# ishine/minimax-speech

Measured on NVIDIA B200. Metric: audio-sec synthesized/sec (24 kHz), higher is better.
Workload: dtype bf16

## Files before the change

minimax-speech_b200/csrc/kernels.h:

```cpp
#pragma once
#include <atomic>
#include <cstdint>
#include <cuda.h>
#include <cuda_bf16.h>
#include <cuda_runtime.h>

namespace ls {

extern std::atomic<long long> g_launch_count;
extern long long* g_debug_buffer;
extern long long g_debug_bytes;
inline void count_launch() { g_launch_count.fetch_add(1, std::memory_order_relaxed); }

bool pdl_enabled();
bool conv_halo_enabled();
int conv_halo_mode();
bool conv_fuse_res_enabled();
bool conv_dual_enabled();
bool conv_resident_enabled();
bool conv_tma_out_enabled();
template <typename... KArgs, typename... Args>
inline cudaError_t launch_pdl(void (*kernel)(KArgs...), dim3 grid, dim3 block, size_t smem, cudaStream_t stream,
                              int cluster, Args&&... args) {
  cudaLaunchConfig_t cfg = {};
// ... 85 lines not shown
cudaError_t launch_conv_gemm_fp16(const CUtensorMap& mapA0, const CUtensorMap& mapA1, const CUtensorMap& mapW,
                                  const ConvGemmParams& p, int num_sms, cudaStream_t stream);

#ifndef ATTN_KV
#define ATTN_KV 64
#endif
struct AttnParams {
  int B, T, H;
  const int* lengths;
  int chunk;
  float scale_log2e;
  __nv_bfloat16* out;
  const float* bias;
  long long bias_ld, bias_bh;
  long long* timeline;
  long long timeline_entries;
  int fp16;
};
cudaError_t launch_attention(const CUtensorMap& mapQKV, const AttnParams& p, cudaStream_t stream);
cudaError_t launch_attention_fp16(const CUtensorMap& mapQKV, const AttnParams& p, cudaStream_t stream);

#define TBLOCK_VEC_FLOATS 2560
#ifndef TBLOCK_PAIR
#define TBLOCK_PAIR 0
#endif
#if TBLOCK_PAIR
#undef TBLOCK_CLUSTER
#define TBLOCK_CLUSTER 2
#endif
#ifndef TBLOCK_CLUSTER
#define TBLOCK_CLUSTER 1
#endif
#define TBLOCK_WBOX_ROWS (128 / TBLOCK_CLUSTER)
#define TBLOCK_WIDE_BOX_ROWS (TBLOCK_PAIR ? 128 : TBLOCK_WBOX_ROWS)
struct TBlockParams {
  int R;
  int T;
  const int* lengths;
  const float* vec;
  int tail_mode;
  long long* timeline;
  int fp16;
  int no_skip;
};
struct TBlockMaps {
  CUtensorMap att;
  CUtensorMap wo, w1, w2, wqkv;
// ... 47 lines not shown
```

minimax-speech_b200/csrc/ptx.cuh:

```cuda
#pragma once
#include <cstdint>
#include <cuda.h>
#include <cuda_bf16.h>
#include <cuda_fp16.h>
#include <cuda_runtime.h>

#ifndef LS_HALF_FP16
#define LS_HALF_FP16 0
#endif

namespace ls {

__device__ __forceinline__ uint32_t smem_u32(const void* p) {
  return static_cast<uint32_t>(__cvta_generic_to_shared(p));
}

__device__ __forceinline__ void mbar_init(uint64_t* bar, uint32_t count) {
  asm volatile("mbarrier.init.shared::cta.b64 [%0], %1;" ::"r"(smem_u32(bar)), "r"(count) : "memory");
}
__device__ __forceinline__ void fence_barrier_init() {
  asm volatile("fence.mbarrier_init.release.cluster;" ::: "memory");
}
__device__ __forceinline__ void mbar_arrive_expect_tx(uint64_t* bar, uint32_t bytes) {
  asm volatile("mbarrier.arrive.expect_tx.shared::cta.b64 _, [%0], %1;" ::"r"(smem_u32(bar)), "r"(bytes)
// ... 21 lines not shown
#ifdef LS_WAIT_SLEEP_NS
    __nanosleep(LS_WAIT_SLEEP_NS);
#endif
    if ((++spins & 0x3FFu) == 0 && clock64() - t0 > 4000000000LL) __trap();
  }
}

__device__ __forceinline__ void pdl_launch_dependents() { asm volatile("griddepcontrol.launch_dependents;" ::: "memory"); }
__device__ __forceinline__ void pdl_wait() { asm volatile("griddepcontrol.wait;" ::: "memory"); }

template <int N>
__device__ __forceinline__ void reg_dealloc() { asm volatile("setmaxnreg.dec.sync.aligned.u32 %0;" ::"n"(N)); }
template <int N>
__device__ __forceinline__ void reg_alloc() { asm volatile("setmaxnreg.inc.sync.aligned.u32 %0;" ::"n"(N)); }

__device__ __forceinline__ void prefetch_tmap(const CUtensorMap* m) {
  asm volatile("prefetch.tensormap [%0];" ::"l"(reinterpret_cast<uint64_t>(m)) : "memory");
}
__device__ __forceinline__ void tma_prefetch_l2_2d(const CUtensorMap* m, int c0, int c1) {
  asm volatile("cp.async.bulk.prefetch.tensor.2d.L2.global.tile [%0, {%1, %2}];"
               ::"l"(reinterpret_cast<uint64_t>(m)), "r"(c0), "r"(c1)
               : "memory");
}
__device__ __forceinline__ void tma_load_2d(void* dst, const CUtensorMap* m, uint64_t* bar, int c0, int c1) {
  asm volatile(
      "cp.async.bulk.tensor.2d.shared::cluster.global.tile.mbarrier::complete_tx::bytes [%0], [%1, {%3, %4}], [%2];"
      ::"r"(smem_u32(dst)), "l"(reinterpret_cast<uint64_t>(m)), "r"(smem_u32(bar)), "r"(c0), "r"(c1)
      : "memory");
}
__device__ __forceinline__ void tma_load_3d(void* dst, const CUtensorMap* m, uint64_t* bar, int c0, int c1,
                                            int c2) {
  asm volatile(
      "cp.async.bulk.tensor.3d.shared::cluster.global.tile.mbarrier::complete_tx::bytes [%0], [%1, {%3, %4, %5}], [%2];"
      ::"r"(smem_u32(dst)), "l"(reinterpret_cast<uint64_t>(m)), "r"(smem_u32(bar)), "r"(c0), "r"(c1), "r"(c2)
      : "memory");
}
__device__ __forceinline__ void tma_load_2d_mc(void* dst, const CUtensorMap* m, uint64_t* bar, int c0, int c1,
                                               uint16_t cta_mask) {
  asm volatile(
      "cp.async.bulk.tensor.2d.shared::cluster.global.tile.mbarrier::complete_tx::bytes.multicast::cluster "
      "[%0], [%1, {%3, %4}], [%2], %5;"
      ::"r"(smem_u32(dst)), "l"(reinterpret_cast<uint64_t>(m)), "r"(smem_u32(bar)), "r"(c0), "r"(c1), "h"(cta_mask)
      : "memory");
}
__device__ __forceinline__ uint32_t cluster_ctarank() {
  uint32_t r;
// ... 82 lines not shown
               "h"(cta_mask)
               : "memory");
}
__device__ __forceinline__ void tmem_alloc_pair(uint32_t* dst_smem, uint32_t ncols) {
  asm volatile("tcgen05.alloc.cta_group::2.sync.aligned.shared::cta.b32 [%0], %1;" ::"r"(smem_u32(dst_smem)),
               "r"(ncols)
               : "memory");
}
__device__ __forceinline__ void tmem_relinquish_pair() {
  asm volatile("tcgen05.relinquish_alloc_permit.cta_group::2.sync.aligned;" ::: "memory");
}
__device__ __forceinline__ void tmem_dealloc_pair(uint32_t taddr, uint32_t ncols) {
  asm volatile("tcgen05.dealloc.cta_group::2.sync.aligned.b32 %0, %1;" ::"r"(taddr), "r"(ncols) : "memory");
}
__device__ __forceinline__ void umma_bf16_pair(uint32_t tmem_d, uint64_t adesc, uint64_t bdesc, uint32_t idesc,
                                               uint32_t accumulate) {
  asm volatile(
      "{\n\t.reg .pred p;\n\t"
      "setp.ne.b32 p, %4, 0;\n\t"
      "tcgen05.mma.cta_group::2.kind::f16 [%0], %1, %2, %3, p;\n\t}"
      ::"r"(tmem_d), "l"(adesc), "l"(bdesc), "r"(idesc), "r"(accumulate)
      : "memory");
}
__device__ __forceinline__ void umma_commit_pair(uint64_t* bar) {
  asm volatile("tcgen05.commit.cta_group::2.mbarrier::arrive::one.shared::cluster.multicast::cluster.b64 [%0], %1;" ::"r"(
                   smem_u32(bar)),
               "h"((uint16_t)3)
               : "memory");
}
__device__ __forceinline__ uint32_t cluster_addr(const void* p, uint32_t rank) {
  uint32_t r;
  asm volatile("mapa.shared::cluster.u32 %0, %1, %2;" : "=r"(r) : "r"(smem_u32(p)), "r"(rank));
  return r;
}
__device__ __forceinline__ void mbar_arrive_cluster(uint32_t bar_cluster_addr) {
  asm volatile("mbarrier.arrive.release.cluster.shared::cluster.b64 _, [%0];" ::"r"(bar_cluster_addr) : "memory");
}
__device__ __forceinline__ void mbar_arrive_expect_tx_cluster(uint32_t bar_cluster_addr, uint32_t bytes) {
  asm volatile("mbarrier.arrive.expect_tx.release.cluster.shared::cluster.b64 _, [%0], %1;" ::"r"(bar_cluster_addr),
               "r"(bytes)
               : "memory");
}
__device__ __forceinline__ void tma_load_2d_pair(void* dst, const CUtensorMap* m, uint32_t bar_cluster_addr, int c0, int c1) {
  asm volatile(
      "cp.async.bulk.tensor.2d.cta_group::2.shared::cluster.global.tile.mbarrier::complete_tx::bytes [%0], [%1, {%3, %4}], [%2];"
      ::"r"(smem_u32(dst)), "l"(reinterpret_cast<uint64_t>(m)), "r"(bar_cluster_addr), "r"(c0), "r"(c1)
      : "memory");
}
__device__ __forceinline__ void tma_load_3d_pair(void* dst, const CUtensorMap* m, uint32_t bar_cluster_addr, int c0, int c1,
                                                 int c2) {
  asm volatile(
      "cp.async.bulk.tensor.3d.cta_group::2.shared::cluster.global.tile.mbarrier::complete_tx::bytes [%0], [%1, {%3, %4, %5}], [%2];"
      ::"r"(smem_u32(dst)), "l"(reinterpret_cast<uint64_t>(m)), "r"(bar_cluster_addr), "r"(c0), "r"(c1), "r"(c2)
      : "memory");
}
__device__ __forceinline__ bool mbar_try_wait_cluster(uint64_t* bar, uint32_t parity) {
  uint32_t ok;
  asm volatile(
      "{\n\t.reg .pred p;\n\t"
      "mbarrier.try_wait.parity.acquire.cluster.shared::cta.b64 p, [%1], %2;\n\t"
      "selp.u32 %0, 1, 0, p;\n\t}"
      : "=r"(ok)
      : "r"(smem_u32(bar)), "r"(parity)
      : "memory");
  return ok != 0;
}
__device__ __forceinline__ void mbar_wait_cluster(uint64_t* bar, uint32_t parity) {
  const long long t0 = clock64();
  uint32_t spins = 0;
  while (!mbar_try_wait_cluster(bar, parity)) {
    if ((++spins & 0x3FFu) == 0 && clock64() - t0 > 4000000000LL) __trap();
  }
}
__device__ __forceinline__ void tmem_ld_wait() { asm volatile("tcgen05.wait::ld.sync.aligned;" ::: "memory"); }

__device__ __forceinline__ void tmem_ld16(uint32_t taddr, uint32_t (&r)[16]) {
  asm volatile(
      "tcgen05.ld.sync.aligned.32x32b.x16.b32 {%0,%1,%2,%3,%4,%5,%6,%7,%8,%9,%10,%11,%12,%13,%14,%15}, [%16];"
      : "=r"(r[0]), "=r"(r[1]), "=r"(r[2]), "=r"(r[3]), "=r"(r[4]), "=r"(r[5]), "=r"(r[6]), "=r"(r[7]),
        "=r"(r[8]), "=r"(r[9]), "=r"(r[10]), "=r"(r[11]), "=r"(r[12]), "=r"(r[13]), "=r"(r[14]), "=r"(r[15])
      : "r"(taddr)
      : "memory");
}
__device__ __forceinline__ void tmem_ld32(uint32_t taddr, uint32_t (&r)[32]) {
  asm volatile(
      "tcgen05.ld.sync.aligned.32x32b.x32.b32 "
      "{%0,%1,%2,%3,%4,%5,%6,%7,%8,%9,%10,%11,%12,%13,%14,%15,"
      "%16,%17,%18,%19,%20,%21,%22,%23,%24,%25,%26,%27,%28,%29,%30,%31}, [%32];"
      : "=r"(r[0]), "=r"(r[1]), "=r"(r[2]), "=r"(r[3]), "=r"(r[4]), "=r"(r[5]), "=r"(r[6]), "=r"(r[7]),
        "=r"(r[8]), "=r"(r[9]), "=r"(r[10]), "=r"(r[11]), "=r"(r[12]), "=r"(r[13]), "=r"(r[14]), "=r"(r[15]),
        "=r"(r[16]), "=r"(r[17]), "=r"(r[18]), "=r"(r[19]), "=r"(r[20]), "=r"(r[21]), "=r"(r[22]), "=r"(r[23]),
        "=r"(r[24]), "=r"(r[25]), "=r"(r[26]), "=r"(r[27]), "=r"(r[28]), "=r"(r[29]), "=r"(r[30]), "=r"(r[31])
      : "r"(taddr)
      : "memory");
}
// ... 154 lines not shown
```

minimax-speech_b200/csrc/tblock.cu:

```cuda
#include "kernels.h"
#include "profiler.h"
#include "ptx.cuh"

namespace ls {
namespace {

constexpr int kC = 256, kInner = 512, kFF = 1024, kQKV = 1536;
constexpr int kTileM = 128;
constexpr int kSlotBytes = 128 * 64 * 2;
constexpr bool kPair = TBLOCK_PAIR != 0;
constexpr int kRingSlotBytes = kSlotBytes;
#ifndef TBLOCK_SLOTS
#define TBLOCK_SLOTS 5
#endif
constexpr int kSlots = TBLOCK_SLOTS;
#ifndef TBLOCK_PRODUCER_WARPS
#define TBLOCK_PRODUCER_WARPS 3
#endif
constexpr int kProducerWarps = TBLOCK_PRODUCER_WARPS;
constexpr int kMmaWarp = kProducerWarps;
#ifndef TBLOCK_PRODUCER_LANES
#define TBLOCK_PRODUCER_LANES 1
#endif
constexpr int kProducerLanes = TBLOCK_PRODUCER_LANES;
constexpr int kIssuers = kProducerWarps * kProducerLanes;
static_assert(kIssuers <= kSlots, "interleaved producers must not outnumber the ring slots (parity waits)");
static_assert(!kPair || TBLOCK_CLUSTER == 2, "pair mode is a cluster of two");
constexpr int kCS = TBLOCK_CLUSTER;
constexpr int kPartRows = 128 / kCS;
constexpr int kPartBytes = kPartRows * 128;
constexpr uint16_t kCtaMask = (uint16_t)((1u << kCS) - 1);
#ifndef TBLOCK_RING_B
#define TBLOCK_RING_B 0
#endif
constexpr bool kRingB = TBLOCK_RING_B != 0 && !kPair && kCS == 1;
#ifndef TBLOCK_WIDE_FF
#define TBLOCK_WIDE_FF 0
#endif
#ifndef TBLOCK_FF2_TS
#define TBLOCK_FF2_TS 1
#endif
constexpr bool kFf2Ts = TBLOCK_FF2_TS != 0 && !kPair;
#ifndef TBLOCK_DETAIL_TL
#define TBLOCK_DETAIL_TL 0
#endif
constexpr bool kDetailTl = TBLOCK_DETAIL_TL != 0;
#ifndef TBLOCK_MERGE_ELECT
#define TBLOCK_MERGE_ELECT 0
#endif
constexpr bool kMergeElect = TBLOCK_MERGE_ELECT != 0;
#ifndef TBLOCK_L2_PREFETCH
#define TBLOCK_L2_PREFETCH 1
#endif
constexpr bool kL2Prefetch = TBLOCK_L2_PREFETCH != 0 && !kPair && kCS == 1;
#ifndef TBLOCK_ATT_DIRECT
#define TBLOCK_ATT_DIRECT 1
#endif
constexpr bool kAttDirect = TBLOCK_ATT_DIRECT != 0 && !kPair && kCS == 1 && !kRingB;
constexpr int kOutLoads = kAttDirect ? 16 : 24;
constexpr bool kWide = TBLOCK_WIDE_FF != 0 && kAttDirect && kFf2Ts && kSlots == 5 && !kMergeElect;
constexpr int kWideSlots = 9;
constexpr int kWideAhPerTile = 26;
static_assert(!kRingB || kFf2Ts, "the second ring lives in the AH region: it needs the TS form of FF2");
constexpr int kSlotsB = 4;
constexpr int kEpiWarps = 16;
constexpr int kEpiThreads = kEpiWarps * 32;
constexpr int kFirstEpiWarp = kProducerWarps + 1;
constexpr int kThreads = kFirstEpiWarp * 32 + kEpiThreads;

constexpr int kOffA3 = 0;
constexpr int kOffAH = 4 * kSlotBytes;
constexpr int kOffRing = kOffAH + 4 * kSlotBytes;
constexpr int kOffVec = kOffRing + kSlots * kRingSlotBytes;
constexpr int kOffRed = kOffVec + TBLOCK_VEC_FLOATS * 4;
constexpr int kOffBars = kOffRed + 4 * kTileM * 8;
constexpr int kBarBytes = 1024;
constexpr int kSmemBytes = kOffBars + kBarBytes + 1024;
static_assert(kSmemBytes <= 227 * 1024, "tblock shared memory budget");

constexpr int V_BO = 0, V_G3 = 256, V_BE3 = 512, V_B1 = 768, V_B2 = 1792, V_G1N = 2048, V_BE1N = 2304;
static_assert(V_BE1N + 256 == TBLOCK_VEC_FLOATS, "vector pack layout");

constexpr uint32_t kTmemD = 0, kTmemH = 256;
// ... 107 lines not shown
  const int n_groups = (n_tiles + kCS - 1) / kCS;
  const int group0 = blockIdx.x / kCS, group_step = gridDim.x / kCS;
  auto group_skipped = [&](int g) {
    for (int r = 0; r < kCS; ++r)
      if (!tile_all_padding(p, (g * kCS + r) * kTileM)) return false;
    return true;
  };
  long long* tl = p.timeline ? p.timeline + (size_t)blockIdx.x * 256 : nullptr;
#define TL(i)                         \
  do {                                \
    if (tl) tl[(i)] = clock64();      \
  } while (0)

  if (warp == 0 && lane == 0) {
    prefetch_tmap(&mapAtt);
    prefetch_tmap(&mapWo);
    prefetch_tmap(&mapW1);
    prefetch_tmap(&mapW2);
    prefetch_tmap(&mapWqkv);
    prefetch_tmap(&mapU);
    prefetch_tmap(&mapQkvOut);
    prefetch_tmap(&mapTail);
    for (int i = 0; i < kWideSlots; ++i) {
      mbar_init(&full[i], kPair ? 2 : 1);
      mbar_init(&empty[i], kPair ? 1 : kCS);
      mbar_init(&empty[kWideSlots + i], 1);
    }
    mbar_init(d_full, 1);
    mbar_init(a3_ready, kPair ? 2 * kEpiWarps : kEpiWarps);
    for (int i = 0; i < 2; ++i) {
      mbar_init(&h_full[i], 1);
      mbar_init(&ah_ready[i], kPair ? 2 * kEpiWarps : kEpiWarps);
      mbar_init(&ah_free[i], 1);
    }
    mbar_init(u_full, 1);
    for (int i = 0; i < kSlotsB; ++i) {
      mbar_init(&full_b[i], 1);
      mbar_init(&empty_b[i], 1);
    }
    mbar_init(stage_free, 1);
    for (int i = 0; i < 8; ++i) {
      mbar_init(&full_c[i], 1);
      mbar_init(&empty_c[i], 1);
    }
    fence_barrier_init();
  }
  if (kL2Prefetch && warp == 1 && lane == 0) {
    const int n_boxes = head ? 48 : (do_qkv ? 128 : 80);
    for (int j = blockIdx.x; j < n_boxes; j += gridDim.x) {
      int q = j;
      if (head || q >= 80) {
        if (!head) q -= 80;
        tma_prefetch_l2_2d(&mapWqkv, (q & 3) * 64, (q >> 2) * 128);
      } else if (q < 16) {
        tma_prefetch_l2_2d(&mapWo, (q >> 1) * 64, (q & 1) * 128);
      } else if (q < 48) {
        q -= 16;
        tma_prefetch_l2_2d(&mapW1, (q & 3) * 64, (q >> 2) * 128);
      } else {
        q -= 48;
        tma_prefetch_l2_2d(&mapW2, (q >> 1) * 64, (q & 1) * 128);
      }
    }
  }
  if (warp == kMmaWarp) {
    __syncwarp();
    if (kPair) {
      tmem_alloc_pair(tmem_slot, 512);
      tmem_relinquish_pair();
    } else {
      tmem_alloc(tmem_slot, 512);
      tmem_relinquish();
    }
  }
  if (warp >= kFirstEpiWarp) {
    for (int i = threadIdx.x - kFirstEpiWarp * 32; i < TBLOCK_VEC_FLOATS; i += kEpiThreads) sVec[i] = __ldg(p.vec + i);
  }
  pdl_launch_dependents();
  tc_fence_before();
  __syncthreads();
  if (kCS > 1) cluster_sync_all();
  tc_fence_after();
  const uint32_t tmem_base = *tmem_slot;
  pdl_wait();

  if (warp < kProducerWarps) {
    constexpr bool kWarpIssue = kProducerLanes == 1;
    if (kWarpIssue || lane < kProducerLanes) {
      const int issuer = warp * kProducerLanes + (kWarpIssue ? 0 : lane);
      const int per_tile = kPair ? (head ? 24 : (do_qkv ? 72 : 48)) : (head ? 48 : (do_qkv ? kOutLoads + 112 : kOutLoads + 64));
      long long seq0 = 0;
      uint32_t tile_n = 0;
      for (int g = group0; g < n_groups; g += group_step) {
        const int row0 = (g * kCS + rank) * kTileM;
        if (kWarpIssue ? __shfl_sync(0xffffffffu, (int)group_skipped(g), 0) != 0 : group_skipped(g)) continue;
        const bool two_rings = kRingB && !head;
        const bool b_warp = two_rings && warp == kProducerWarps - 1;
        const int n_a = two_rings ? kIssuers - kProducerLanes : kIssuers;
        for (int i = two_rings ? 0 : issuer; i < per_tile; i += two_rings ? 1 : kIssuers) {
          const CUtensorMap* m;
          int c0, c1;
          bool own_rows = false;
          int c2 = -1;
          int ring_b = -1, chunk_b = 0;
          int a_idx = i;
          if (kPair) {
            auto chunk_half = [&](const CUtensorMap* wm, int chunk, int half) {
              m = wm, c0 = 0, c1 = chunk * 128 + rank * kPartRows, c2 = half * 2;
            };
            if (head) {
              chunk_half(&mapWqkv, i >> 1, i & 1);
            } else if (i < 16) {
              const int kb = i >> 1;
              if ((i & 1) == 0) m = &mapAtt, c0 = kb * 64, c1 = row0, own_rows = true;
              else m = &mapWo, c0 = kb * 64, c1 = rank * 128, own_rows = true;
            } else if (i < 20) {
              chunk_half(&mapW1, (i - 16) >> 1, i & 1);
            } else if (i < 48) {
              const int j = i - 20;
              int c, r;
              if (j < 24) c = j >> 2, r = j & 3;
              else c = 6 + ((j - 24) >> 1), r = (j - 24) & 1;
              if (r < 2) m = &mapW2, c0 = c * 128 + r * 64, c1 = rank * 128, own_rows = true;
              else chunk_half(&mapW1, c + 2, r - 2);
            } else {
              chunk_half(&mapWqkv, (i - 48) >> 1, i & 1);
            }
          } else if (head) {
            m = &mapWqkv, c0 = (i & 3) * 64, c1 = (i >> 2) * 128;
          } else if (kAttDirect && i < kOutLoads) {
            m = &mapWo, c0 = (i >> 1) * 64, c1 = (i & 1) * 128;
          } else if (i < kOutLoads) {
            const int kb = i / 3, r = i - kb * 3;
            if (r == 0) m = &mapAtt, c0 = kb * 64, c1 = row0, own_rows = true;
            else m = &mapWo, c0 = kb * 64, c1 = (r - 1) * 128;
          } else if (i < kOutLoads + 8) {
            const int j = i - kOutLoads;
            m = &mapW1, c0 = (j & 3) * 64, c1 = (j >> 2) * 128;
          } else if (i < kOutLoads + 64) {
            const int j = i - (kOutLoads + 8);
            int c, r;
            if (j < 48) c = j >> 3, r = j & 7;
            else c = 6 + ((j - 48) >> 2), r = (j - 48) & 3;
            if (r < 4) {
              m = &mapW2, c0 = c * 128 + (r >> 1) * 64, c1 = (r & 1) * 128;
              if (kRingB) ring_b = r, chunk_b = c;
            } else {
              m = &mapW1, c0 = (r - 4) * 64, c1 = (c + 2) * 128;
            }
// ... 24 lines not shown
              if (hc < 4) mbar_wait(stage_free, tile_n & 1);
            } else {
              const uint32_t cnt = tile_n * (uint32_t)(per_tile - (head ? 0 : kWideAhPerTile)) + (uint32_t)rc;
              sl = 4 + (int)(cnt % 5u), use = cnt / 5u;
            }
            if (use > 0) mbar_wait(&empty[((use - 1) & 1) * kWideSlots + sl], ((use - 1) >> 1) & 1);
            if (tl && i < 48 && tile_n == 0 && (!kWarpIssue || lane == 0)) tl[64 + i] = clock64();
            full_bar = &full[sl];
            dst = sAH + sl * kSlotBytes;
          } else if (ring_b >= 0) {
            if (chunk_b == 0) mbar_wait(stage_free, tile_n & 1);
            else mbar_wait(&empty_b[ring_b], (tile_n * 7 + (uint32_t)chunk_b - 1) & 1);
            full_bar = &full_b[ring_b];
            dst = sAH + ring_b * kSlotBytes;
          } else {
            const long long seq = seq0 + a_idx;
            const int slot = (int)(seq % kSlots);
            const uint32_t use = (uint32_t)(seq / kSlots);
            mbar_wait(&empty[slot], (use & 1) ^ 1);
            if (tl && seq < 48 && (!kWarpIssue || lane == 0)) tl[64 + seq] = clock64();
            full_bar = &full[slot];
            dst = sRing + slot * kRingSlotBytes;
          }
          const int qk6 = kOutLoads + 64 + 24;
          const bool stamp_q6 = kDetailTl && tl && !kWide && do_qkv && !head && i >= qk6 && i < qk6 + 4 && seq0 == 0;
          if (stamp_q6 && (!kWarpIssue || lane == 0)) tl[216 + 2 * (i - qk6)] = clock64();
          if (kWarpIssue && !elect_one()) {
          } else if (kPair) {
            const uint32_t fb = cluster_addr(full_bar, 0);
            mbar_arrive_expect_tx_cluster(fb, kRingSlotBytes);
            if (c2 >= 0) tma_load_3d_pair(dst, m, fb, c0, c1, c2);
            else tma_load_2d_pair(dst, m, fb, c0, c1);
          } else {
            mbar_arrive_expect_tx(full_bar, kSlotBytes);
            if (kCS > 1 && !own_rows) tma_load_2d_mc(dst + rank * kPartBytes, m, full_bar, c0, c1 + rank * kPartRows, kCtaMask);
            else tma_load_2d(dst, m, full_bar, c0, c1);
          }
          if (kWarpIssue) __syncwarp();
          if (stamp_q6 && (!kWarpIssue || lane == 0)) tl[217 + 2 * (i - qk6)] = clock64();
        }
        seq0 += (kRingB && !head) ? per_tile - 32 : per_tile;
        tile_n += 1;
      }
    }
  } else if (warp == kMmaWarp) {
    if (!kPair || rank == 0) {
      const uint32_t tmem_u = __shfl_sync(0xffffffffu, tmem_base, 0);
#define TLM(i)                                 \
  do {                                         \
    if (tl && lane == 0) tl[(i)] = clock64();  \
  } while (0)
      const uint32_t idesc = make_idesc_bf16(kPair ? 2 * kTileM : kTileM, 128, false, false);
      const uint32_t idesc256 = make_idesc_bf16(2 * kTileM, 256, false, false);
      auto mma = [&](uint32_t d, uint64_t ad, uint64_t bd, uint32_t acc) {
        if (kPair) umma_bf16_pair(d, ad, bd, idesc, acc);
        else umma_bf16(d, ad, bd, idesc, acc);
      };
      auto commit = [&](uint64_t* bar) {
        if (elect_one()) {
          if (kPair) umma_commit_pair(bar);
          else umma_commit(bar);
        }
        __syncwarp();
      };
      auto wait_epi = [&](uint64_t* bar, uint32_t parity) {
        if (kPair) mbar_wait_cluster(bar, parity);
        else mbar_wait(bar, parity);
      };
      int slot = 0;
      uint32_t phase = 0;
      uint32_t a3_cnt = 0;
      uint32_t fills0 = 0, fills1 = 0;
      uint32_t drained0 = 0, drained1 = 0;
      int n_full = 0;
      uint32_t tile_n = 0;
      int r_slot = 0, h_slot = 0, f_pos = 0;
      uint32_t r_use = 0, h_use = 0;
      bool in_f = false;
      auto wide_peek = [&](int ahead, uint32_t& use) -> int {
        int rs = r_slot, hs = h_slot, fp = f_pos;
        uint32_t ru = r_use, hu = h_use;
        for (int a = 0;; ++a) {
          const bool ah = in_f && fp < 4;
          if (a == ahead) {
            use = ah ? hu : ru;
            return ah ? hs : 4 + rs;
          }
          if (ah) {
            if (++hs == 4) hs = 0, ++hu;
          } else {
            if (++rs == 5) rs = 0, ++ru;
// ... 4 lines not shown
      auto wide_advance = [&](int n) {
        for (int a = 0; a < n; ++a) {
          if (in_f && f_pos < 4) {
            if (++h_slot == 4) h_slot = 0, ++h_use;
          } else {
            if (++r_slot == 5) r_slot = 0, ++r_use;
          }
          if (in_f && ++f_pos == 9) f_pos = 0;
        }
      };
      auto slot_desc = [&](int ahead) -> uint64_t {
        if (kWide) {
          uint32_t use;
          const int sl = wide_peek(ahead, use);
          mbar_wait(&full[sl], use & 1);
          tc_fence_after();
          if (tl && lane == 0 && n_full < 16) tl[112 + n_full] = clock64();
          n_full += (ahead == 0);
          return make_smem_desc_sw128(smem_u32(sAH + sl * kSlotBytes));
        }
        int s = slot + ahead;
        uint32_t ph = phase;
        if (s >= kSlots) s -= kSlots, ph ^= 1;
        if (kPair) mbar_wait_cluster(&full[s], ph);
        else mbar_wait(&full[s], ph);
        tc_fence_after();
        if (tl && lane == 0 && n_full < 16) tl[112 + n_full] = clock64();
        n_full += (ahead == 0);
        return make_smem_desc_sw128(smem_u32(sRing + s * kRingSlotBytes));
      };
      auto release = [&](int n) {
        if (kWide) {
          if (elect_one()) {
            for (int j = 0; j < n; ++j) {
              uint32_t use;
              const int sl = wide_peek(j, use);
              umma_commit(&empty[(use & 1) * kWideSlots + sl]);
            }
          }
          __syncwarp();
          wide_advance(n);
          return;
        }
        if (elect_one()) {
          int sl = slot;
          for (int j = 0; j < n; ++j) {
            if (kPair) umma_commit_pair(&empty[sl]);
            else if (kCS > 1) umma_commit_mc(&empty[sl], kCtaMask);
// ... 2 lines not shown
          }
        }
        __syncwarp();
        for (int j = 0; j < n; ++j)
          if (++slot == kSlots) slot = 0, phase ^= 1;
      };
      auto release_elected = [&](int n) {
        int sl = slot;
        for (int j = 0; j < n; ++j) {
          if (kPair) umma_commit_pair(&empty[sl]);
          else if (kCS > 1) umma_commit_mc(&empty[sl], kCtaMask);
          else umma_commit(&empty[sl]);
          if (++sl == kSlots) sl = 0;
        }
      };
      auto advance = [&](int n) {
        __syncwarp();
        for (int j = 0; j < n; ++j)
          if (++slot == kSlots) slot = 0, phase ^= 1;
      };
      auto wait_drained = [&](int i) {
        const uint32_t f = i ? fills1 : fills0;
        if ((i ? drained1 : drained0) < f) {
          wait_epi(&ah_ready[i], (f - 1) & 1);
          tc_fence_after();
          if (i) drained1 = f;
          else drained0 = f;
        }
      };
      auto gemm_from_a3 = [&](int i, int tlb = -1) {
        if (kDetailTl && tl && tlb >= 0 && lane == 0) tl[tlb] = clock64();
        wait_drained(i);
        if (kDetailTl && tl && tlb >= 0 && lane == 0) tl[tlb + 1] = clock64();
        const uint32_t d = tmem_u + kTmemH + (uint32_t)i * 128;
        for (int kb = 0; kb < kC / 64; ++kb) {
          const uint64_t bdesc = slot_desc(0) + (kPair ? (uint64_t)((kb & 1) * (8192 >> 4)) : 0);
          if (kDetailTl && tl && tlb >= 0 && lane == 0) tl[tlb + 2 + kb] = clock64();
          const uint64_t adesc = make_smem_desc_sw128(smem_u32(sA3 + kb * kSlotBytes));
          if (kMergeElect && !kPair) {
            if (elect_one()) {
#pragma unroll
              for (int k = 0; k < 4; ++k) mma(d, adesc + 2 * k, bdesc + 2 * k, (kb | k) != 0 ? 1u : 0u);
              release_elected(1);
            }
            advance(1);
            continue;
          }
// ... 4 lines not shown
          if (kDetailTl && tl && tlb >= 0 && lane == 0) tl[tlb + 56 + 2 * kb] = clock64();
          if (!kPair || (kb & 1)) release(1);
          if (kDetailTl && tl && tlb >= 0 && lane == 0) tl[tlb + 57 + 2 * kb] = clock64();
        }
        commit(&h_full[i]);
        if (kDetailTl && tl && tlb >= 0 && lane == 0) tl[tlb + 6] = clock64();
        if (i) fills1 += 1;
        else fills0 += 1;
      };
      const uint32_t dD = tmem_u + kTmemD;
      TLM(0);
      for (int g = group0; g < n_groups; g += group_step, ++tile_n) {
        if (__shfl_sync(0xffffffffu, (int)group_skipped(g), 0)) {
          --tile_n;
          continue;
        }
        if (g != group0) tl = nullptr;
        if (!head) {
        for (int kb = 0; kb < kInner / 64; ++kb) {
          if (kAttDirect) {
            mbar_wait(&full_c[kb], tile_n & 1);
            tc_fence_after();
            const uint64_t adesc = make_smem_desc_sw128(smem_u32(att_place(kb)));
            const uint64_t b0 = slot_desc(0);
            const uint64_t b1 = slot_desc(1);
            if (kb == 0) TLM(1);
            if (elect_one()) {
#pragma unroll
              for (int k = 0; k < 4; ++k) {
                const uint32_t acc = (kb | k) != 0 ? 1u : 0u;
                mma(dD, adesc + 2 * k, b0 + 2 * k, acc);
                mma(dD + 128, adesc + 2 * k, b1 + 2 * k, acc);
              }
              if (!kWide) release_elected(2);
              umma_commit(&empty_c[kb]);
            }
            if (kWide) release(2);
            else advance(2);
            continue;
          }
          const uint64_t adesc = slot_desc(0);
          const uint64_t b0 = slot_desc(1);
          if (kPair) {
            if (kb == 0) TLM(1);
            if (elect_one()) {
#pragma unroll
              for (int k = 0; k < 4; ++k) umma_bf16_pair(dD, adesc + 2 * k, b0 + 2 * k, idesc256, (kb | k) != 0 ? 1u : 0u);
            }
            release(2);
            continue;
          }
          const uint64_t b1 = slot_desc(2);
          if (kb == 0) TLM(1);
          if (elect_one()) {
#pragma unroll
            for (int k = 0; k < 4; ++k) {
              const uint32_t acc = (kb | k) != 0 ? 1u : 0u;
              mma(dD, adesc + 2 * k, b0 + 2 * k, acc);
              mma(dD + 128, adesc + 2 * k, b1 + 2 * k, acc);
            }
            if (kMergeElect) release_elected(3);
          }
          if (kMergeElect) advance(3);
          else release(3);
        }
        commit(d_full);
        TLM(2);
        wait_epi(a3_ready, a3_cnt & 1);
        a3_cnt += 1;
        tc_fence_after();
        TLM(3);
        gemm_from_a3(0);
        gemm_from_a3(1);
        in_f = true, f_pos = 0;
        for (int c = 0; c < kFF / 128; ++c) {
          const int i = c & 1;
          if (kDetailTl && c == 4) TLM(128);
          wait_drained(i);
          TLM(4 + c);
          for (int kb2 = 0; kb2 < 2; ++kb2) {
            const uint32_t a_tm = tmem_u + kTmemH + (uint32_t)i * 128 + (uint32_t)kb2 * 64;
            const uint64_t adesc = make_smem_desc_sw128(smem_u32(sAH + i * 2 * kSlotBytes + kb2 * kSlotBytes));
            if (kPair) {
              const uint64_t b0 = slot_desc(0);
              if (elect_one()) {
#pragma unroll
                for (int k = 0; k < 4; ++k) umma_bf16_pair(dD, adesc + 2 * k, b0 + 2 * k, idesc256, 1u);
              }
              release(1);
              continue;
            }
            uint64_t b0, b1;
            if (kRingB) {
              const uint32_t par = (tile_n * 8 + (uint32_t)c) & 1;
              mbar_wait(&full_b[2 * kb2], par);
              if (kDetailTl && c == 4) TLM(129 + 2 * kb2);
              mbar_wait(&full_b[2 * kb2 + 1], par);
              tc_fence_after();
              b0 = make_smem_desc_sw128(smem_u32(sAH + (2 * kb2) * kSlotBytes));
              b1 = make_smem_desc_sw128(smem_u32(sAH + (2 * kb2 + 1) * kSlotBytes));
            } else {
              b0 = slot_desc(0);
              if (kDetailTl && c == 4) TLM(129 + 2 * kb2);
              b1 = slot_desc(1);
            }
            if (kDetailTl && c == 4) TLM(130 + 2 * kb2);
            if (elect_one()) {
#pragma unroll
              for (int k = 0; k < 4; ++k) {
                if (kFf2Ts) {
                  const uint32_t a_k = a_tm + (uint32_t)(k >> 1) * 32 + (uint32_t)(k & 1) * 8;
                  umma_bf16_ts(dD, a_k, b0 + 2 * k, idesc, 1u);
                  umma_bf16_ts(dD + 128, a_k, b1 + 2 * k, idesc, 1u);
                } else {
                  mma(dD, adesc + 2 * k, b0 + 2 * k, 1u);
                  mma(dD + 128, adesc + 2 * k, b1 + 2 * k, 1u);
                }
              }
              if (kRingB && c + 1 < kFF / 128) umma_commit(&empty_b[2 * kb2]), umma_commit(&empty_b[2 * kb2 + 1]);
              if (!kRingB && kMergeElect) release_elected(2);
            }
            if (kRingB) __syncwarp();
            else if (kMergeElect) advance(2);
            else release(2);
          }
          if (!kFf2Ts) commit(&ah_free[i]);
          if (kDetailTl && c == 4) TLM(133);
          if (c + 2 < kFF / 128) gemm_from_a3(i, kDetailTl && c == 4 ? 134 : -1);
        }
        in_f = false;
        commit(d_full);
        TLM(12);
        }
        wait_epi(a3_ready, a3_cnt & 1);
        a3_cnt += 1;
        tc_fence_after();
        TLM(13);
        if (do_qkv)
          for (int c = 0; c < kQKV / 128; ++c) {
            gemm_from_a3(c & 1, kDetailTl && c == 6 ? 144 : -1);
            TLM(14 + c);
          }
        TLM(26);
      }
    }
  } else {
#undef TLM
    const int q = warp & 3;
    const int cg = (warp - kFirstEpiWarp) >> 2;
    const int row = q * 32 + lane;
    const int sw = row & 7;
    const bool leader = threadIdx.x == kFirstEpiWarp * 32;
    const uint32_t trow = tmem_base + ((uint32_t)(q * 32) << 16);
    uint8_t* stage = sAH;
    uint32_t d_cnt = 0, u_cnt = 0;
    uint32_t h_cnt0 = 0, h_cnt1 = 0;
    uint32_t ah_cnt0 = 0, ah_cnt1 = 0;
    auto warp_arrive = [&](uint64_t* bar) {
      fence_proxy_async_smem();
      tc_fence_before();
      __syncwarp();
      if (lane == 0) {
        if (kPair) mbar_arrive_cluster(cluster_addr(bar, 0));
        else mbar_arrive(bar);
      }
    };
    for (int g = group0; g < n_groups; g += group_step) {
      const int row0 = (g * kCS + rank) * kTileM;
      if (group_skipped(g)) continue;
      const int grow = row0 + row;
      bool valid = grow < p.R;
      if (valid && p.lengths) {
        const int b = grow / p.T;
        valid = grow - b * p.T < p.lengths[b];
      }
      long long* tle = (leader && g == group0) ? tl : nullptr;
#define TLE(i)                        \
  do {                                \
    if (tle) tle[(i)] = clock64();    \
  } while (0)
      if (warp == kFirstEpiWarp) {
        if (leader) {
          bulk_wait_read<0>();
          mbar_arrive_expect_tx(u_full, 8 * kSlotBytes);
        }
        __syncwarp();
        if (kAttDirect && !head) {
          if (lane < 8) {
            mbar_arrive_expect_tx(&full_c[lane], kSlotBytes);
            tma_load_2d(att_place(lane), &mapAtt, &full_c[lane], lane * 64, row0);
          }
          __syncwarp();
          if (lane == 0) {
            for (int j = 0; j < 8; ++j) {
              mbar_wait(&empty_c[j], u_cnt & 1);
              tma_load_2d(att_place(j), &mapU, u_full, j * 32, row0);
            }
          }
          __syncwarp();
        } else if (lane < 8) {
          tma_load_2d(att_place(lane), &mapU, u_full, lane * 32, row0);
        }
      }

      {
        mbar_wait(u_full, u_cnt & 1);
        u_cnt += 1;
        if (!head) {
          mbar_wait(d_full, d_cnt & 1);
          d_cnt += 1;
        }
        tc_fence_after();
        TLE(32);
// ... 102 lines not shown
        for (int k = 0; k < 8; ++k) {
          const float4 b2 = reinterpret_cast<const float4*>(sVec + V_B2 + col)[k];
          x[4 * k + 0] += b2.x;
          x[4 * k + 1] += b2.y;
          x[4 * k + 2] += b2.z;
          x[4 * k + 3] += b2.w;
        }
      };
      if (head) {
        epi_barrier();
      } else if (!do_qkv) {
#pragma unroll 1
        for (int ch = 0; ch < 2; ++ch) {
          float x[32];
          load_u2(ch, x);
          if (!valid) {
#pragma unroll
            for (int k = 0; k < 32; ++k) x[k] = 0.f;
          }
          store_row_chunks(stage + cg * kSlotBytes + row * 128, sw, ch * 4, x);
        }
        warp_arrive(a3_ready);
        epi_barrier();
        if (leader) {
#pragma unroll
          for (int k = 0; k < 4; ++k) tma_store_2d(&mapTail, stage + k * kSlotBytes, k * 64, row0);
          bulk_commit();
        }
      } else {
        auto stage_u = [&](const float (&v)[32]) {
          uint8_t* dst = stage + cg * kSlotBytes + row * 128;
#pragma unroll
          for (int k = 0; k < 8; ++k)
            *reinterpret_cast<float4*>(dst + ((k ^ sw) << 4)) = make_float4(v[4 * k], v[4 * k + 1], v[4 * k + 2], v[4 * k + 3]);
          fence_proxy_async_smem();
        };
        auto store_u = [&](int ch) {
#pragma unroll
          for (int k = 0; k < 4; ++k) tma_store_2d(&mapU, stage + k * kSlotBytes, k * 64 + ch * 32, row0);
          bulk_commit();
        };
        RowStats st;
#pragma unroll 1
        for (int ch = 0; ch < 2; ++ch) {
          float x[32];
          load_u2(ch, x);
          st.add32(x);
          tmem_st32(trow + kTmemD + cg * 64 + ch * 32, reinterpret_cast<const uint32_t(&)[32]>(x));
          if (ch == 0) stage_u(x);
        }
        tmem_st_wait();
        float mean, rstd;
        combine_groups(st, sRed, cg, row, mean, rstd);
        if (leader) store_u(0);
        const float nmr = -mean * rstd;
#pragma unroll 1
        for (int ch = 0; ch < 2; ++ch) {
          const int col = cg * 64 + ch * 32;
          float x[32];
          tmem_ld32(trow + kTmemD + col, reinterpret_cast<uint32_t(&)[32]>(x));
// ... 19 lines not shown
        epi_barrier();
      }
      if (do_qkv) {
        for (int c = 0; c < kQKV / 128; ++c) {
          const int i = c & 1;
          if (kDetailTl && c == 6) TLE(170);
          mbar_wait(&h_full[i], (i ? h_cnt1 : h_cnt0) & 1);
          if (i) h_cnt1 += 1;
          else h_cnt0 += 1;
          tc_fence_after();
          if (kDetailTl && c == 6) TLE(171);
          float y[32];
          tmem_ld32(trow + kTmemH + i * 128 + cg * 32, reinterpret_cast<uint32_t(&)[32]>(y));
          tmem_ld_wait();
          warp_arrive(&ah_ready[i]);
          if (kDetailTl && c == 6) TLE(172);
          store_row_chunks(stage + (i * 2 + (cg >> 1)) * kSlotBytes + row * 128, sw, (cg & 1) * 4, y);
          fence_proxy_async_smem();
          if (kDetailTl && c == 6) TLE(173);
          if (leader) bulk_wait_read<0>();
          if (kDetailTl && c == 6) TLE(174);
          epi_barrier();
          if (kDetailTl && c == 6) TLE(175);
          if (leader) {
            tma_store_2d(&mapQkvOut, stage + (i * 2 + 0) * kSlotBytes, c * 128, row0);
            tma_store_2d(&mapQkvOut, stage + (i * 2 + 1) * kSlotBytes, c * 128 + 64, row0);
            bulk_commit();
          }
          if (kDetailTl && c == 6) TLE(176);
          TLE(44 + c);
        }
      }
    }
    if (leader) bulk_wait<0>();
  }

  tc_fence_before();
  __syncthreads();
  if (kCS > 1) cluster_sync_all();
  if (warp == kMmaWarp) {
    tc_fence_after();
    if (kPair) tmem_dealloc_pair(tmem_base, 512);
    else tmem_dealloc(tmem_base, 512);
  }
}

}
// ... 41 lines not shown
```

profiles/timeline_tblock.py:

```python
import os
import sys

sys.path.insert(0, os.path.dirname(os.path.dirname(os.path.abspath(__file__))))
import torch

import minimax_speech_b200.native as native
import profiles.time_kernels as tk

DEV = torch.device("cuda:0")
lib = native.load()
buf = torch.zeros(148 * 256, dtype=torch.int64, device=DEV)
R = int(os.environ.get("LS_R", "16000"))
tk.tblock(R, 0)
lib.ls_debug_set_buffer(native.ptr(buf), buf.numel() * 8)
tk.tblock(R, 0)
lib.ls_debug_set_buffer(None, 0)
t = buf.view(148, 256).cpu()
for cta in (0, 60, 124):
    r = t[cta]
    base = int(r[0])
    names = {0: "start", 1: "P1 first slots", 2: "P1 issued", 3: "a3_ready#1", 12: "FF issued", 13: "a3_ready#2", 26: "end"}
    print(f"--- CTA {cta}  (cycles since MMA-thread start)")
    print("MMA :", " ".join(f"{names.get(i, str(i))}={int(r[i]) - base}" for i in range(0, 27) if int(r[i])))
    print("EPI :", " ".join(f"{i}={int(r[i]) - base}" for i in range(32, 56) if int(r[i])))
    print("LOAD slot-free time of loads 0..47:", [int(r[64 + i]) - base if int(r[64 + i]) else None for i in range(48)])
    print("MMA saw slots 0..15 full at:", [int(r[112 + i]) - base for i in range(16)])
    d = lambda a, b: [int(r[i]) - base if int(r[i]) else None for i in range(a, b)]
    print("MMA FF chunk 4: before AH wait, after, kb2=0 slot0/slot1, kb2=1 slot0/slot1... :", d(128, 134))
    print("MMA FF1(6): before drained wait, after, kb0..3 slot seen, committed:", d(134, 141))
    print("MMA QKV chunk 6: before drained wait, after, kb0..3 slot seen, committed:", d(144, 151))
    print("EPI FF chunk 4: before h_full, after, ld done, gelu done, ah_free ok, arrived:", d(160, 166))
    print("EPI out-proj LayerNorm (leader thread): pass 1 chunk 0 / 1 done, tmem_st drained, statistics combined, pass 2 chunk 0 / 1 done:", d(56, 62))
    print("LOAD QKV chunk 6, boxes 0..3: (slot free seen by the producer, TMA issued):", d(216, 224))
    print("MMA QKV chunk 6, kb0..3: (MMAs issued, commit issued):", d(200, 208))
    print("EPI QKV chunk 6: before h_full, after, ld+arrive, staged, bulk_wait_read, barrier, stores issued:", d(170, 177))
```

Before: 2350.

## Enable 2-CTA pair mode for transformer block with TS FF2 and direct attention loads

Turns on the paired-CTA (cta_group::2) transformer block by default and reworks the pair path so it uses the attention-direct layout, TMEM-sourced A operand for FF2, and L2 weight prefetch. Barrier handling is simplified: only rank 0 sets the expected transaction bytes for both CTAs, and cluster-scope waits are replaced by local waits. Padding-only tiles skip their stores. The change is meant to halve per-CTA weight traffic and feed wider MMAs, at the cost of cluster coupling and more complex synchronisation.

```diff
diff --git a/minimax-speech_b200/csrc/kernels.h b/minimax-speech_b200/csrc/kernels.h
--- a/minimax-speech_b200/csrc/kernels.h
+++ b/minimax-speech_b200/csrc/kernels.h
@@ -131,7 +131,7 @@
 
 #define TBLOCK_VEC_FLOATS 2560
 #ifndef TBLOCK_PAIR
-#define TBLOCK_PAIR 0
+#define TBLOCK_PAIR 1
 #endif
 #if TBLOCK_PAIR
 #undef TBLOCK_CLUSTER
diff --git a/minimax-speech_b200/csrc/ptx.cuh b/minimax-speech_b200/csrc/ptx.cuh
--- a/minimax-speech_b200/csrc/ptx.cuh
+++ b/minimax-speech_b200/csrc/ptx.cuh
@@ -67,6 +67,11 @@
                ::"l"(reinterpret_cast<uint64_t>(m)), "r"(c0), "r"(c1)
                : "memory");
 }
+__device__ __forceinline__ void tma_prefetch_l2_3d(const CUtensorMap* m, int c0, int c1, int c2) {
+  asm volatile("cp.async.bulk.prefetch.tensor.3d.L2.global.tile [%0, {%1, %2, %3}];"
+               ::"l"(reinterpret_cast<uint64_t>(m)), "r"(c0), "r"(c1), "r"(c2)
+               : "memory");
+}
 __device__ __forceinline__ void tma_load_2d(void* dst, const CUtensorMap* m, uint64_t* bar, int c0, int c1) {
   asm volatile(
       "cp.async.bulk.tensor.2d.shared::cluster.global.tile.mbarrier::complete_tx::bytes [%0], [%1, {%3, %4}], [%2];"
@@ -195,6 +200,15 @@
       ::"r"(tmem_d), "l"(adesc), "l"(bdesc), "r"(idesc), "r"(accumulate)
       : "memory");
 }
+__device__ __forceinline__ void umma_bf16_pair_ts(uint32_t tmem_d, uint32_t tmem_a, uint64_t bdesc, uint32_t idesc,
+                                                  uint32_t accumulate) {
+  asm volatile(
+      "{\n\t.reg .pred p;\n\t"
+      "setp.ne.b32 p, %4, 0;\n\t"
+      "tcgen05.mma.cta_group::2.kind::f16 [%0], [%1], %2, %3, p;\n\t}"
+      ::"r"(tmem_d), "r"(tmem_a), "l"(bdesc), "r"(idesc), "r"(accumulate)
+      : "memory");
+}
 __device__ __forceinline__ void umma_commit_pair(uint64_t* bar) {
   asm volatile("tcgen05.commit.cta_group::2.mbarrier::arrive::one.shared::cluster.multicast::cluster.b64 [%0], %1;" ::"r"(
                    smem_u32(bar)),
@@ -206,13 +220,8 @@
   asm volatile("mapa.shared::cluster.u32 %0, %1, %2;" : "=r"(r) : "r"(smem_u32(p)), "r"(rank));
   return r;
 }
-__device__ __forceinline__ void mbar_arrive_cluster(uint32_t bar_cluster_addr) {
-  asm volatile("mbarrier.arrive.release.cluster.shared::cluster.b64 _, [%0];" ::"r"(bar_cluster_addr) : "memory");
-}
-__device__ __forceinline__ void mbar_arrive_expect_tx_cluster(uint32_t bar_cluster_addr, uint32_t bytes) {
-  asm volatile("mbarrier.arrive.expect_tx.release.cluster.shared::cluster.b64 _, [%0], %1;" ::"r"(bar_cluster_addr),
-               "r"(bytes)
-               : "memory");
+__device__ __forceinline__ void mbar_arrive_remote(uint32_t bar_cluster_addr) {
+  asm volatile("mbarrier.arrive.shared::cluster.b64 _, [%0];" ::"r"(bar_cluster_addr) : "memory");
 }
 __device__ __forceinline__ void tma_load_2d_pair(void* dst, const CUtensorMap* m, uint32_t bar_cluster_addr, int c0, int c1) {
   asm volatile(
@@ -226,24 +235,6 @@
       "cp.async.bulk.tensor.3d.cta_group::2.shared::cluster.global.tile.mbarrier::complete_tx::bytes [%0], [%1, {%3, %4, %5}], [%2];"
       ::"r"(smem_u32(dst)), "l"(reinterpret_cast<uint64_t>(m)), "r"(bar_cluster_addr), "r"(c0), "r"(c1), "r"(c2)
       : "memory");
-}
-__device__ __forceinline__ bool mbar_try_wait_cluster(uint64_t* bar, uint32_t parity) {
-  uint32_t ok;
-  asm volatile(
-      "{\n\t.reg .pred p;\n\t"
-      "mbarrier.try_wait.parity.acquire.cluster.shared::cta.b64 p, [%1], %2;\n\t"
-      "selp.u32 %0, 1, 0, p;\n\t}"
-      : "=r"(ok)
-      : "r"(smem_u32(bar)), "r"(parity)
-      : "memory");
-  return ok != 0;
-}
-__device__ __forceinline__ void mbar_wait_cluster(uint64_t* bar, uint32_t parity) {
-  const long long t0 = clock64();
-  uint32_t spins = 0;
-  while (!mbar_try_wait_cluster(bar, parity)) {
-    if ((++spins & 0x3FFu) == 0 && clock64() - t0 > 4000000000LL) __trap();
-  }
 }
 __device__ __forceinline__ void tmem_ld_wait() { asm volatile("tcgen05.wait::ld.sync.aligned;" ::: "memory"); }
 
diff --git a/minimax-speech_b200/csrc/tblock.cu b/minimax-speech_b200/csrc/tblock.cu
--- a/minimax-speech_b200/csrc/tblock.cu
+++ b/minimax-speech_b200/csrc/tblock.cu
@@ -40,7 +40,7 @@
 #ifndef TBLOCK_FF2_TS
 #define TBLOCK_FF2_TS 1
 #endif
-constexpr bool kFf2Ts = TBLOCK_FF2_TS != 0 && !kPair;
+constexpr bool kFf2Ts = TBLOCK_FF2_TS != 0;
 #ifndef TBLOCK_DETAIL_TL
 #define TBLOCK_DETAIL_TL 0
 #endif
@@ -52,13 +52,14 @@
 #ifndef TBLOCK_L2_PREFETCH
 #define TBLOCK_L2_PREFETCH 1
 #endif
-constexpr bool kL2Prefetch = TBLOCK_L2_PREFETCH != 0 && !kPair && kCS == 1;
+constexpr bool kL2Prefetch = TBLOCK_L2_PREFETCH != 0 && (kPair || kCS == 1);
 #ifndef TBLOCK_ATT_DIRECT
 #define TBLOCK_ATT_DIRECT 1
 #endif
-constexpr bool kAttDirect = TBLOCK_ATT_DIRECT != 0 && !kPair && kCS == 1 && !kRingB;
-constexpr int kOutLoads = kAttDirect ? 16 : 24;
-constexpr bool kWide = TBLOCK_WIDE_FF != 0 && kAttDirect && kFf2Ts && kSlots == 5 && !kMergeElect;
+constexpr bool kAttDirect = TBLOCK_ATT_DIRECT != 0 && (kPair || kCS == 1) && !kRingB;
+static_assert(!kPair || (kAttDirect && kFf2Ts), "pair mode is built on the att-direct layout and the TS form of FF2");
+constexpr int kOutLoads = kPair ? 8 : (kAttDirect ? 16 : 24);
+constexpr bool kWide = TBLOCK_WIDE_FF != 0 && !kPair && kAttDirect && kFf2Ts && kSlots == 5 && !kMergeElect;
 constexpr int kWideSlots = 9;
 constexpr int kWideAhPerTile = 26;
 static_assert(!kRingB || kFf2Ts, "the second ring lives in the AH region: it needs the TS form of FF2");
@@ -212,7 +213,7 @@
     prefetch_tmap(&mapQkvOut);
     prefetch_tmap(&mapTail);
     for (int i = 0; i < kWideSlots; ++i) {
-      mbar_init(&full[i], kPair ? 2 : 1);
+      mbar_init(&full[i], 1);
       mbar_init(&empty[i], kPair ? 1 : kCS);
       mbar_init(&empty[kWideSlots + i], 1);
     }
@@ -237,16 +238,19 @@
   }
   if (kL2Prefetch && warp == 1 && lane == 0) {
     const int n_boxes = head ? 48 : (do_qkv ? 128 : 80);
+    auto prefetch_chunked = [&](const CUtensorMap* wm, int q) {
+      if (kPair) tma_prefetch_l2_3d(wm, 0, (q >> 1) * 64, (q & 1) * 2);
+      else tma_prefetch_l2_2d(wm, (q & 3) * 64, (q >> 2) * 128);
+    };
     for (int j = blockIdx.x; j < n_boxes; j += gridDim.x) {
       int q = j;
       if (head || q >= 80) {
         if (!head) q -= 80;
-        tma_prefetch_l2_2d(&mapWqkv, (q & 3) * 64, (q >> 2) * 128);
+        prefetch_chunked(&mapWqkv, q);
       } else if (q < 16) {
         tma_prefetch_l2_2d(&mapWo, (q >> 1) * 64, (q & 1) * 128);
       } else if (q < 48) {
-        q -= 16;
-        tma_prefetch_l2_2d(&mapW1, (q & 3) * 64, (q >> 2) * 128);
+        prefetch_chunked(&mapW1, q - 16);
       } else {
         q -= 48;
         tma_prefetch_l2_2d(&mapW2, (q >> 1) * 64, (q & 1) * 128);
@@ -278,7 +282,8 @@
     constexpr bool kWarpIssue = kProducerLanes == 1;
     if (kWarpIssue || lane < kProducerLanes) {
       const int issuer = warp * kProducerLanes + (kWarpIssue ? 0 : lane);
-      const int per_tile = kPair ? (head ? 24 : (do_qkv ? 72 : 48)) : (head ? 48 : (do_qkv ? kOutLoads + 112 : kOutLoads + 64));
+      const int per_tile = kPair ? (head ? 24 : (do_qkv ? kOutLoads + 56 : kOutLoads + 32))
+                                 : (head ? 48 : (do_qkv ? kOutLoads + 112 : kOutLoads + 64));
       long long seq0 = 0;
       uint32_t tile_n = 0;
       for (int g = group0; g < n_groups; g += group_step) {
@@ -300,21 +305,19 @@
             };
             if (head) {
               chunk_half(&mapWqkv, i >> 1, i & 1);
-            } else if (i < 16) {
-              const int kb = i >> 1;
-              if ((i & 1) == 0) m = &mapAtt, c0 = kb * 64, c1 = row0, own_rows = true;
-              else m = &mapWo, c0 = kb * 64, c1 = rank * 128, own_rows = true;
-            } else if (i < 20) {
-              chunk_half(&mapW1, (i - 16) >> 1, i & 1);
-            } else if (i < 48) {
-              const int j = i - 20;
+            } else if (i < kOutLoads) {
+              m = &mapWo, c0 = i * 64, c1 = rank * 128;
+            } else if (i < kOutLoads + 4) {
+              chunk_half(&mapW1, (i - kOutLoads) >> 1, i & 1);
+            } else if (i < kOutLoads + 32) {
+              const int j = i - (kOutLoads + 4);
               int c, r;
               if (j < 24) c = j >> 2, r = j & 3;
               else c = 6 + ((j - 24) >> 1), r = (j - 24) & 1;
-              if (r < 2) m = &mapW2, c0 = c * 128 + r * 64, c1 = rank * 128, own_rows = true;
+              if (r < 2) m = &mapW2, c0 = c * 128 + r * 64, c1 = rank * 128;
               else chunk_half(&mapW1, c + 2, r - 2);
             } else {
-              chunk_half(&mapWqkv, (i - 48) >> 1, i & 1);
+              chunk_half(&mapWqkv, (i - (kOutLoads + 32)) >> 1, i & 1);
             }
           } else if (head) {
             m = &mapWqkv, c0 = (i & 3) * 64, c1 = (i >> 2) * 128;
@@ -385,13 +388,13 @@
             full_bar = &full[slot];
             dst = sRing + slot * kRingSlotBytes;
           }
-          const int qk6 = kOutLoads + 64 + 24;
+          const int qk6 = kPair ? kOutLoads + 32 + 12 : kOutLoads + 64 + 24;
           const bool stamp_q6 = kDetailTl && tl && !kWide && do_qkv && !head && i >= qk6 && i < qk6 + 4 && seq0 == 0;
           if (stamp_q6 && (!kWarpIssue || lane == 0)) tl[216 + 2 * (i - qk6)] = clock64();
           if (kWarpIssue && !elect_one()) {
           } else if (kPair) {
+            if (rank == 0) mbar_arrive_expect_tx(full_bar, 2 * kRingSlotBytes);
             const uint32_t fb = cluster_addr(full_bar, 0);
-            mbar_arrive_expect_tx_cluster(fb, kRingSlotBytes);
             if (c2 >= 0) tma_load_3d_pair(dst, m, fb, c0, c1, c2);
             else tma_load_2d_pair(dst, m, fb, c0, c1);
           } else {
@@ -426,10 +429,6 @@
         }
         __syncwarp();
       };
-      auto wait_epi = [&](uint64_t* bar, uint32_t parity) {
-        if (kPair) mbar_wait_cluster(bar, parity);
-        else mbar_wait(bar, parity);
-      };
       int slot = 0;
       uint32_t phase = 0;
       uint32_t a3_cnt = 0;
@@ -480,8 +479,7 @@
         int s = slot + ahead;
         uint32_t ph = phase;
         if (s >= kSlots) s -= kSlots, ph ^= 1;
-        if (kPair) mbar_wait_cluster(&full[s], ph);
-        else mbar_wait(&full[s], ph);
+        mbar_wait(&full[s], ph);
         tc_fence_after();
         if (tl && lane == 0 && n_full < 16) tl[112 + n_full] = clock64();
         n_full += (ahead == 0);
@@ -530,7 +528,7 @@
       auto wait_drained = [&](int i) {
         const uint32_t f = i ? fills1 : fills0;
         if ((i ? drained1 : drained0) < f) {
-          wait_epi(&ah_ready[i], (f - 1) & 1);
+          mbar_wait(&ah_ready[i], (f - 1) & 1);
           tc_fence_after();
           if (i) drained1 = f;
           else drained0 = f;
@@ -581,6 +579,18 @@
             mbar_wait(&full_c[kb], tile_n & 1);
             tc_fence_after();
             const uint64_t adesc = make_smem_desc_sw128(smem_u32(att_place(kb)));
+            if (kPair) {
+              const uint64_t b0 = slot_desc(0);
+              if (kb == 0) TLM(1);
+              if (elect_one()) {
+#pragma unroll
+                for (int k = 0; k < 4; ++k) umma_bf16_pair(dD, adesc + 2 * k, b0 + 2 * k, idesc256, (kb | k) != 0 ? 1u : 0u);
+                release_elected(1);
+                umma_commit_pair(&empty_c[kb]);
+              }
+              advance(1);
+              continue;
+            }
             const uint64_t b0 = slot_desc(0);
             const uint64_t b1 = slot_desc(1);
             if (kb == 0) TLM(1);
@@ -600,15 +610,6 @@
           }
           const uint64_t adesc = slot_desc(0);
           const uint64_t b0 = slot_desc(1);
-          if (kPair) {
-            if (kb == 0) TLM(1);
-            if (elect_one()) {
-#pragma unroll
-              for (int k = 0; k < 4; ++k) umma_bf16_pair(dD, adesc + 2 * k, b0 + 2 * k, idesc256, (kb | k) != 0 ? 1u : 0u);
-            }
-            release(2);
-            continue;
-          }
           const uint64_t b1 = slot_desc(2);
           if (kb == 0) TLM(1);
           if (elect_one()) {
@@ -625,7 +626,7 @@
         }
         commit(d_full);
         TLM(2);
-        wait_epi(a3_ready, a3_cnt & 1);
+        mbar_wait(a3_ready, a3_cnt & 1);
         a3_cnt += 1;
         tc_fence_after();
         TLM(3);
@@ -642,9 +643,11 @@
             const uint64_t adesc = make_smem_desc_sw128(smem_u32(sAH + i * 2 * kSlotBytes + kb2 * kSlotBytes));
             if (kPair) {
               const uint64_t b0 = slot_desc(0);
+              if (kDetailTl && c == 4) TLM(130 + 2 * kb2);
               if (elect_one()) {
 #pragma unroll
-                for (int k = 0; k < 4; ++k) umma_bf16_pair(dD, adesc + 2 * k, b0 + 2 * k, idesc256, 1u);
+                for (int k = 0; k < 4; ++k)
+                  umma_bf16_pair_ts(dD, a_tm + (uint32_t)(k >> 1) * 32 + (uint32_t)(k & 1) * 8, b0 + 2 * k, idesc256, 1u);
               }
               release(1);
               continue;
@@ -691,7 +694,7 @@
         commit(d_full);
         TLM(12);
         }
-        wait_epi(a3_ready, a3_cnt & 1);
+        mbar_wait(a3_ready, a3_cnt & 1);
         a3_cnt += 1;
         tc_fence_after();
         TLM(13);
@@ -720,7 +723,7 @@
       tc_fence_before();
       __syncwarp();
       if (lane == 0) {
-        if (kPair) mbar_arrive_cluster(cluster_addr(bar, 0));
+        if (kPair) mbar_arrive_remote(cluster_addr(bar, 0));
         else mbar_arrive(bar);
       }
     };
@@ -733,6 +736,7 @@
         const int b = grow / p.T;
         valid = grow - b * p.T < p.lengths[b];
       }
+      const bool storer = leader && !(kPair && tile_all_padding(p, row0));
       long long* tle = (leader && g == group0) ? tl : nullptr;
 #define TLE(i)                        \
   do {                                \
@@ -746,8 +750,13 @@
         __syncwarp();
         if (kAttDirect && !head) {
           if (lane < 8) {
-            mbar_arrive_expect_tx(&full_c[lane], kSlotBytes);
-            tma_load_2d(att_place(lane), &mapAtt, &full_c[lane], lane * 64, row0);
+            if (kPair) {
+              if (rank == 0) mbar_arrive_expect_tx(&full_c[lane], 2 * kSlotBytes);
+              tma_load_2d_pair(att_place(lane), &mapAtt, cluster_addr(&full_c[lane], 0), lane * 64, row0);
+            } else {
+              mbar_arrive_expect_tx(&full_c[lane], kSlotBytes);
+              tma_load_2d(att_place(lane), &mapAtt, &full_c[lane], lane * 64, row0);
+            }
           }
           __syncwarp();
           if (lane == 0) {
@@ -896,7 +905,7 @@
         }
         warp_arrive(a3_ready);
         epi_barrier();
-        if (leader) {
+        if (storer) {
 #pragma unroll
           for (int k = 0; k < 4; ++k) tma_store_2d(&mapTail, stage + k * kSlotBytes, k * 64, row0);
           bulk_commit();
@@ -910,6 +919,7 @@
           fence_proxy_async_smem();
         };
         auto store_u = [&](int ch) {
+          if (!storer) return;
 #pragma unroll
           for (int k = 0; k < 4; ++k) tma_store_2d(&mapU, stage + k * kSlotBytes, k * 64 + ch * 32, row0);
           bulk_commit();
@@ -975,7 +985,7 @@
           if (kDetailTl && c == 6) TLE(174);
           epi_barrier();
           if (kDetailTl && c == 6) TLE(175);
-          if (leader) {
+          if (storer) {
             tma_store_2d(&mapQkvOut, stage + (i * 2 + 0) * kSlotBytes, c * 128, row0);
             tma_store_2d(&mapQkvOut, stage + (i * 2 + 1) * kSlotBytes, c * 128 + 64, row0);
             bulk_commit();
diff --git a/profiles/timeline_tblock.py b/profiles/timeline_tblock.py
--- a/profiles/timeline_tblock.py
+++ b/profiles/timeline_tblock.py
@@ -16,7 +16,7 @@
 tk.tblock(R, 0)
 lib.ls_debug_set_buffer(None, 0)
 t = buf.view(148, 256).cpu()
-for cta in (0, 60, 124):
+for cta in [int(c) for c in os.environ.get("LS_CTAS", "0,60,124").split(",")]:
     r = t[cta]
     base = int(r[0])
     names = {0: "start", 1: "P1 first slots", 2: "P1 issued", 3: "a3_ready#1", 12: "FF issued", 13: "a3_ready#2", 26: "end"}
```

After: 2498 (median of 6 runs). 6.3% higher.
